# thethomasboyer/PhenDiff

Hardware: AMD Instinct MI355X
Metric: img2img images/sec (50-step DDIM invert+denoise, 256x256) (higher is better)
Workload: dtype bf16; 1 GPU; configs[2]: 256x256 pipeline_conditional_ddim invert->class-swap->denoise, 50+50 DDIM steps, super_small UNet (random init, seed 0), 3k_steps_clipping_rescaling, 32 images/GPU/step sharded over 1 GPU(s), no collectives; batch_per_gpu=32, global_batch=32, inference_steps=50, image_size=256, hipgraph=True, concurrent_trajectories=1

## Files before the change

### phendiff_amd/csrc/conv_igemm.hip

```cpp
#include <type_traits>
#include <utility>
#include <stdio.h>
#include <stdlib.h>
#include "pd_common.h"
#include "pd_stage.h"
#include "pd_conv.h"

namespace pd {

constexpr int CONV_AR8 = 6;
constexpr int CONV_PRO_DEFAULT = 1;
constexpr int CONV_PRO_WPS = 3;
constexpr int CONV_PRO_START = 8;
template <int... I, typename F> __device__ __forceinline__ void pd_static_for_impl(std::integer_sequence<int, I...>, F&& f) { (f(std::integral_constant<int, I>{}), ...); }
template <int N, typename F> __device__ __forceinline__ void pd_static_for(F&& f) { pd_static_for_impl(std::make_integer_sequence<int, N>{}, f); }
constexpr int PRO_OPS = 37;
constexpr int pro_op_cost(int k) {
  if (k >= 36) return 100;
  const int stg = (k % 18) >> 1;
  return (stg == 3 || stg == 4 || stg == 6 || stg == 7) ? 87 : (stg == 0 ? 60 : (stg == 8 ? 106 : 58));
}
constexpr int pro_ops_done(int S, int NS, int PS0, int NIT) {
  if (S < PS0) return 0;
  if (S >= NS - 1) return NIT * PRO_OPS;
  long long tot = 0;
  for (int k = 0; k < PRO_OPS; ++k) tot += pro_op_cost(k);
  tot *= NIT;
  const long long target = (long long)(S - PS0 + 1) * tot / (NS - PS0);
  int done = 0;
  long long dc = 0;
  while (done < NIT * PRO_OPS && dc + pro_op_cost(done % PRO_OPS) <= target) { dc += pro_op_cost(done % PRO_OPS); ++done; }
  return done;
}
__device__ __forceinline__ unsigned pd_lin_block() { return blockIdx.x + gridDim.x * (blockIdx.y + gridDim.y * blockIdx.z); }
template <typename T, int KS, int STRIDE, int TH, int TW, bool DB, bool TAIL, int NCO = 1, bool PLAIN = false, int PRO = 0, bool STACK = false>
__global__ __launch_bounds__(256, NCO == 2 ? 2 : (PRO ? CONV_PRO_WPS : (((KS == 1 || (KS == 3 && STRIDE == 1 && TH * TW == 256)) && sizeof(T) == 2) ? 3 : 2))) void conv_kernel(const ConvP p) {
  static_assert(PRO == 0 || (!PLAIN && DB && KS == 3 && STRIDE == 1 && sizeof(T) == 2), "compile-time prologue: 16-bit 3x3 stride-1 double-buffered launches");
  static_assert(!TAIL || (DB && KS == 3 && STRIDE == 1), "fused shortcut tail: 3x3 stride-1 double-buffered variant only");
  static_assert(NCO == 1 || (NCO == 2 && DB && KS == 3 && STRIDE == 1), "two output tiles per workgroup: 3x3 stride-1 double-buffered variant only");
  static_assert(!STACK || (KS == 3 && STRIDE == 1 && TW == 8 && TH == 16 && NCO == 1 && !PLAIN && PRO == 0), "stacked 8 x 8 images: the 16 x 8 tile");
  constexpr int SG = STACK ? TH / 8 : 1;
  using E = Elem<T>;
  using Frag = typename E::Frag;
  using SR = typename Stage<T>::R;
  constexpr int TP = TH * TW;
  constexpr int NF = TP / 64;
  constexpr int RPF = 32 / TW;
  constexpr int IN_TH = STACK ? SG * 10 : (TH - 1) * STRIDE + KS;
  constexpr int IN_TW = (TW - 1) * STRIDE + KS;
  constexpr int NPIX = IN_TH * IN_TW;
  constexpr bool M16 = PLAIN && sizeof(T) == 2 && (KS == 3 || KS == 2) && STRIDE == 1 && DB && TW >= 16;
  constexpr int CHB = 32 * E::BYTES;
  constexpr int PITCH = DB ? 2 * CHB + (M16 ? 32 : 16) : CHB + 16;
  constexpr int NIT = (NPIX * 4 + 255) / 256;
  constexpr int TAPS = KS * KS;
  constexpr int KSTEPS = TAPS * 2;
  constexpr int LDS_TILE = DB ? CHB : 0;
  static_assert(RPF >= 1 && TW * RPF == 32, "TW must divide 32");

  extern __shared__ __attribute__((aligned(16))) unsigned char lds[];

  int co_t = blockIdx.y, n = blockIdx.z * SG, bx = blockIdx.x;
  if (!STACK && p.co_major) {
    const int gx = gridDim.x, gxz = gridDim.x * gridDim.z;
    const int idx = xcd_chunk_index((int)pd_lin_block(), gxz * (int)gridDim.y);
    co_t = idx / gxz;
    const int rem = idx - co_t * gxz;
    n = rem / gx; bx = rem - n * gx;
  }
  int tx, ty;
  if (p.tiles_x_shift >= 0) { tx = bx & (p.tiles_x - 1); ty = bx >> p.tiles_x_shift; }
  else { ty = bx / p.tiles_x; tx = bx - ty * p.tiles_x; }
  const int y0 = ty * TH, x0 = tx * TW;

  const int tid = threadIdx.x;
  const int lane = tid & 63;
  const int wave = __builtin_amdgcn_readfirstlane(tid >> 6);
  const int wp = wave >> 1, wc = wave & 1;
  const int r = lane & 31, h = lane >> 5;
  const int ct32 = co_t * (2 * NCO) + wc;
  const bool wave_active = (ct32 * 32) < p.Cout_pad;

  const __amdgpu_buffer_rsrc_t rs0 = __builtin_amdgcn_make_buffer_rsrc((void*)p.x0, 0, p.bytes0, 0x00020000);
  const __amdgpu_buffer_rsrc_t rs1 = __builtin_amdgcn_make_buffer_rsrc((void*)(p.x1 ? p.x1 : p.x0), 0, p.bytes1, 0x00020000);

  const __amdgpu_buffer_rsrc_t rt0 = __builtin_amdgcn_make_buffer_rsrc((void*)(TAIL ? p.t0 : p.x0), 0, TAIL ? p.tbytes0 : p.bytes0, 0x00020000);
  const __amdgpu_buffer_rsrc_t rt1 = __builtin_amdgcn_make_buffer_rsrc((void*)((TAIL && p.t1) ? p.t1 : p.x0), 0, (TAIL && p.t1) ? p.tbytes1 : p.bytes0, 0x00020000);

  const int sub = tid & 3;
  auto stage_pix = [&](int i) { return (tid + 256 * i) >> 2; };
  const int Hc = p.upsample ? p.Hin * 2 : p.Hin;
  const int Wc = p.upsample ? p.Win * 2 : p.Win;
  int spix[NIT];
  constexpr int TAIL_CENTRE = 1 << 30;
  const int ups = p.upsample ? 1 : 0;
  const int ph_mask = p.upsample >= 2 ? 1 : 0, ph_want = p.upsample == 3 ? 1 : 0;
  const int istep = p.in_step, Ws = p.Win * istep;
  const int iy_base = y0 * STRIDE - p.pad, ix_base = x0 * STRIDE - p.pad_x, n_base = n * p.Hin * istep + p.in_oy;
#pragma unroll
  for (int i = 0; i < NIT; ++i) {
    const int pix = stage_pix(i);
    const int u = pix / IN_TW, vv = pix - u * IN_TW;
    const int sj = STACK ? u / 10 : 0, su = u - sj * 10;
    const int iy = STACK ? su - 1 : iy_base + u, ix = ix_base + vv;
    const bool ok = (pix < NPIX) & ((unsigned)iy < (unsigned)Hc) & ((unsigned)ix < (unsigned)Wc) & (!STACK || n + sj < p.B)
                    & (((iy & ph_mask) == (ph_want & ph_mask)) & ((ix & ph_mask) == (ph_want & ph_mask)));
    int v = STACK ? ((n + sj) * 8 + iy) * 8 + ix : (n_base + (iy >> ups) * istep) * Ws + (ix >> ups) * istep + p.in_ox;
    if (TAIL) v |= (((unsigned)((STACK ? su : u) - KS / 2) < (unsigned)(STACK ? 8 : TH)) & ((unsigned)(vv - KS / 2) < (unsigned)TW)) ? TAIL_CENTRE : 0;
    spix[i] = ok ? v : -1;
  }
  const bool affine = PRO || (!PLAIN && p.scale != nullptr);
  const bool do_silu = PRO || (!PLAIN && p.silu != 0);
  const int cin = p.C0 + p.C1;

  SR stage[NIT];
  float sc[8], sh[8];
  bool stage_plain = false;
  auto issue_loads = [&](int chunk) {
    int src, cch;
    if (!TAIL || chunk < p.n_main) { cch = chunk * 32; src = cch < p.C0 ? 0 : 1; if (src == 1) cch -= p.C0; }
    else { cch = (chunk - p.n_main) * 32; src = cch < p.Ct0 ? 2 : 3; if (src == 3) cch -= p.Ct0; }
    stage_plain = TAIL && src >= 2;
    const unsigned cs = src == 0 ? p.C0 : (src == 1 ? p.C1 : (src == 2 ? p.Ct0 : p.Ct1));
    const unsigned cbytes = (unsigned)(cch + sub * 8) * E::BYTES;
#pragma unroll
    for (int i = 0; i < NIT; ++i) {
      const bool want = TAIL ? (stage_plain ? spix[i] >= TAIL_CENTRE : spix[i] >= 0) : spix[i] >= 0;
      const unsigned off = want ? (unsigned)(TAIL ? spix[i] & (TAIL_CENTRE - 1) : spix[i]) * cs * E::BYTES + cbytes : OOB_OFF;
      stage[i] = src == 0 ? Stage<T>::load(rs0, off) : (src == 1 ? Stage<T>::load(rs1, off)
                 : (src == 2 ? Stage<T>::load(rt0, off) : Stage<T>::load(rt1, off)));
    }
    if ((PRO && !stage_plain) || (!PRO && affine && !stage_plain)) {
      const int cg = chunk * 32 + sub * 8;
      const float* ps = p.scale + (size_t)n * cin + cg;
      const float* pb = p.shift + (size_t)n * cin + cg;
      const f32x4 a0 = *(const f32x4*)ps, a1 = *((const f32x4*)ps + 1);
      const f32x4 b0 = *(const f32x4*)pb, b1 = *((const f32x4*)pb + 1);
#pragma unroll
      for (int j = 0; j < 4; ++j) { sc[j] = a0[j]; sc[4 + j] = a1[j]; sh[j] = b0[j]; sh[4 + j] = b1[j]; }
    }
  };
  auto write_piece = [&](int i, unsigned char* buf, bool tail_piece = false) {
    const int pix = stage_pix(i);
    if constexpr (PRO) {
      if (TAIL && tail_piece) {
        if (pix < NPIX && spix[i] >= 0) *(u32x4*)(buf + pix * PITCH + sub * 8 * E::BYTES) = Stage<T>::raw(stage[i]);
        return;
      }
      const u32x4 o = Stage<T>::xform_gs(stage[i], sc, sh);
      const bool ok = pix < NPIX && spix[i] >= 0;
      *(u32x4*)(ok ? buf + pix * PITCH + sub * 8 * E::BYTES : lds + NPIX * PITCH) = o;
    } else
    if (pix < NPIX && spix[i] >= 0)
      Stage<T>::template xform_store<false>(buf + pix * PITCH + sub * 8 * E::BYTES, stage[i], sc, sh, affine && !stage_plain,
                                            do_silu && !stage_plain, true);
  };
  auto zero_padding = [&]() {
#pragma unroll
    for (int i = 0; i < NIT; ++i) {
      const int pix = stage_pix(i);
      if (pix < NPIX && spix[i] < 0) {
        unsigned char* d = lds + pix * PITCH + sub * 8 * E::BYTES;
#pragma unroll
        for (int q = 0; q < (DB ? 2 : 1); ++q)
#pragma unroll
          for (int b16 = 0; b16 < 8 * E::BYTES; b16 += 16) *(u32x4*)(d + q * LDS_TILE + b16) = (u32x4)(0u);
      }
    }
  };

  auto stage_im2col = [&](unsigned char* buf) {
    if constexpr (KS == 1 && STRIDE == 1) {
      const int py = tid / TW, px = tid % TW;
      const int oy = y0 + py, ox = x0 + px;
// ... 17 lines not shown
      }
#pragma unroll
      for (int q = 0; q < 4; ++q) {
        float o[8];
#pragma unroll
        for (int j = 0; j < 8; ++j) o[j] = v[q * 8 + j];
        E::store(buf + tid * PITCH + q * 8 * E::BYTES, E::pack(o));
      }
    }
  };

  auto frag_row = [&](int fi, int q) { return fi * RPF + q; };
  const int li = lane & 15, lg = lane >> 4;
  constexpr int TJ_STEP = (TW >= 32 ? 16 : IN_TW) * PITCH;
  int rbase[NF];
#pragma unroll
  for (int f = 0; f < NF; ++f) {
    const int fi = wp * NF + f;
    if constexpr (M16) {
      rbase[f] = f == 0 ? ((wp * NF * RPF) * IN_TW + li) * PITCH + lg * 8 * E::BYTES : 0;
    } else {
      const int py = frag_row(fi, r / TW), px = r % TW;
      const int ly = STACK ? py + 2 * (py >> 3) : py * STRIDE;
      rbase[f] = (ly * IN_TW + px * STRIDE) * PITCH + h * 8 * E::BYTES;
    }
  }

  f32x16 acc[NCO][NF];
  f32x4 acq[NCO][NF][4];
  const int main_ksteps = (TAIL ? p.n_main : p.nchunks) * KSTEPS;
  const int all_ksteps = main_ksteps + (TAIL ? p.n_tail * 2 : 0);
  const unsigned wfrag = 512u * E::BYTES;
  const __amdgpu_buffer_rsrc_t rw = __builtin_amdgcn_make_buffer_rsrc((void*)p.w, 0, (unsigned)(p.Cout_pad / 32) * (unsigned)all_ksteps * wfrag, 0x00020000);
  const unsigned wlane = (unsigned)lane * 8u * E::BYTES;
  const unsigned wtile = (unsigned)ct32 * (unsigned)all_ksteps * wfrag;
  const unsigned wstep = 2u * (unsigned)all_ksteps * wfrag;
  auto load_w = [&](int c, int kstep) { return E::load_buf(rw, wlane, wtile + (unsigned)c * wstep + (unsigned)kstep * wfrag); };

  constexpr int AR = (KS == 3 && TW == 8 && STRIDE == 1 && sizeof(T) == 2 && TP <= 128) ? CONV_AR8 : ((KSTEPS % 3 == 0) ? 3 : 2);
  static_assert(KSTEPS % AR == 0, "the ring index is static");
  constexpr int AD = AR - 1;
  Frag aring[AR][NCO];
  static_assert(!M16 || NF % 2 == 0, "M16 walks a fragment pair per half-step");
  Frag aq[2][NCO][2];
  const unsigned wlane16 = (unsigned)(((lg >> 1) * 64 + (lg & 1) * 32 + li) * 16);
  auto load_w16 = [&](int c, int tap_index, int ti) {
    return E::load_buf(rw, wlane16 + (unsigned)ti * 256u, wtile + (unsigned)c * wstep + (unsigned)(2 * tap_index) * wfrag);
  };

  auto mma_chunk = [&](int chunk, const unsigned char* buf, unsigned char* nbuf, auto have_next_c, auto active_c) {
    constexpr int NEXT = (int)decltype(have_next_c)::value;
    constexpr bool HAVE_NEXT = NEXT != 0, NEXT_PLAIN = NEXT == 2;
    constexpr bool ACTIVE = decltype(active_c)::value;
    const int g0 = chunk * KSTEPS;
    Frag bc[NF];
    int piece = 0;
    if constexpr (!PRO) __builtin_amdgcn_iglp_opt(0);
    if constexpr (PRO && ACTIVE) {
      constexpr int NM = NCO * NF;
      constexpr int NS = KSTEPS * NM;
      constexpr int PS0 = CONV_PRO_START < NS - 8 ? CONV_PRO_START : 0;
      f32x2 py[4], pw[4];
      u32x4 po;
      auto piece_op = [&](auto ic, auto kc) __attribute__((always_inline)) {
        constexpr int i = decltype(ic)::value, k = decltype(kc)::value;
        if constexpr (k < 36) {
          constexpr int half = k / 18, kk = k % 18, stg = kk >> 1, j = half * 2 + (kk & 1);
          if constexpr (stg == 0) { const uint32_t wj = Stage<T>::word(stage[i], j); float lo, hi; Pack16<T>::unpack(wj, lo, hi); pw[j].x = lo; pw[j].y = hi; }
          else if constexpr (stg == 1) py[j] = pw[j] * (f32x2){sc[2 * j], sc[2 * j + 1]} + (f32x2){sh[2 * j], sh[2 * j + 1]};
          else if constexpr (stg == 2) pw[j] = py[j] * (f32x2)(-1.4426950408889634f);
          else if constexpr (stg == 3) pw[j].x = __builtin_amdgcn_exp2f(pw[j].x);
          else if constexpr (stg == 4) pw[j].y = __builtin_amdgcn_exp2f(pw[j].y);
          else if constexpr (stg == 5) pw[j] = pw[j] + (f32x2)(1.0f);
          else if constexpr (stg == 6) pw[j].x = __builtin_amdgcn_rcpf(pw[j].x);
          else if constexpr (stg == 7) pw[j].y = __builtin_amdgcn_rcpf(pw[j].y);
          else { const f32x2 o = py[j] * pw[j]; po[j] = Pack16<T>::pack(o.x, o.y); }
          if constexpr (stg == 1) asm volatile("" : "+v"(py[j]));
          else if constexpr (stg == 8) { uint32_t w = po[j]; asm volatile("" : "+v"(w)); po[j] = w; }
          else asm volatile("" : "+v"(pw[j]));
        } else {
// ... 145 lines not shown
  };
  using std::true_type; using std::false_type;

  f32x4 bt[NCO][4];
  u32x4 tv[NCO][4];
  if constexpr (M16) {
    if (wave_active) {
      const __amdgpu_buffer_rsrc_t rtemb = __builtin_amdgcn_make_buffer_rsrc((void*)(p.temb ? p.temb : p.bias), 0,
          p.temb ? ((unsigned)n * (unsigned)p.temb_stride + (unsigned)p.Cout) * 4u : 0u, 0x00020000);
#pragma unroll
      for (int c = 0; c < NCO; ++c)
#pragma unroll
        for (int ti = 0; ti < 2; ++ti) {
          const int co = (ct32 + 2 * c) * 32 + 16 * ti + 4 * lg;
          bt[c][ti] = *(const f32x4*)(p.bias + co);
          tv[c][ti] = __builtin_amdgcn_raw_buffer_load_b128(rtemb, (unsigned)(n * p.temb_stride + co) * 4u, 0, 0);
        }
    }
  } else
  if (wave_active) {
    const int nt = STACK ? min(n + wp, p.B - 1) : n;
    const __amdgpu_buffer_rsrc_t rtemb = __builtin_amdgcn_make_buffer_rsrc((void*)(p.temb ? p.temb : p.bias), 0,
        p.temb ? ((unsigned)nt * (unsigned)p.temb_stride + (unsigned)p.Cout) * 4u : 0u, 0x00020000);
#pragma unroll
    for (int c = 0; c < NCO; ++c)
#pragma unroll
      for (int g = 0; g < 4; ++g) {
        const int co = (ct32 + 2 * c) * 32 + 8 * g + 4 * h;
        bt[c][g] = *(const f32x4*)(p.bias + co);
        tv[c][g] = __builtin_amdgcn_raw_buffer_load_b128(rtemb, (unsigned)(nt * p.temb_stride + co) * 4u, 0, 0);
      }
  }
  if (!p.im2col3) issue_loads(0);
  if (wave_active) {
#pragma unroll
    for (int c = 0; c < NCO; ++c)
#pragma unroll
      for (int g = 0; g < (M16 ? 2 : 4); ++g)
#pragma unroll
        for (int i = 0; i < 4; ++i) bt[c][g][i] += __uint_as_float(tv[c][g][i]);
  }
  if constexpr (M16) {
#pragma unroll
    for (int c = 0; c < NCO; ++c)
#pragma unroll
      for (int f = 0; f < NF; ++f)
#pragma unroll
        for (int q = 0; q < 4; ++q) acq[c][f][q] = wave_active ? bt[c][q >> 1] : (f32x4)(0.f);
    if (wave_active) {
#pragma unroll
      for (int c = 0; c < NCO; ++c) { aq[0][c][0] = load_w16(c, 0, 0); aq[0][c][1] = load_w16(c, 0, 1); }
    }
  } else {
#pragma unroll
  for (int c = 0; c < NCO; ++c) {
    f32x16 init = (f32x16)(0.f);
    if (wave_active) {
#pragma unroll
      for (int g = 0; g < 4; ++g)
#pragma unroll
        for (int i = 0; i < 4; ++i) init[4 * g + i] = bt[c][g][i];
    }
#pragma unroll
    for (int f = 0; f < NF; ++f) acc[c][f] = init;
  }
  if (wave_active) {
#pragma unroll
    for (int i = 0; i < AD; ++i)
#pragma unroll
      for (int c = 0; c < NCO; ++c) aring[i][c] = load_w(c, i);
  }
  }
  if (!p.im2col3) zero_padding();
  if (DB) {
    if (p.im2col3) {
      stage_im2col(lds);
    } else {
      write_piece(0, lds);
#pragma unroll
      for (int i = 1; i < NIT; ++i) write_piece(i, lds);
    }
    if (p.nchunks > 1) issue_loads(1);
    __syncthreads();
    int chunk = 0;
    const int main_loop_end = TAIL ? (PRO ? p.n_main - 1 : p.n_main) : p.nchunks - 1;
    for (; chunk < main_loop_end; ++chunk) {
      unsigned char* buf = lds + (chunk & 1) * LDS_TILE;
      unsigned char* nbuf = lds + ((chunk + 1) & 1) * LDS_TILE;
      if constexpr (PRO) mma_chunk(chunk, buf, nbuf, true_type{}, true_type{});
      else if (wave_active) mma_chunk(chunk, buf, nbuf, true_type{}, true_type{});
      else mma_chunk(chunk, buf, nbuf, true_type{}, false_type{});
      if (chunk + 2 < p.nchunks) issue_loads(chunk + 2);
      __syncthreads();
    }
    if constexpr (TAIL && PRO) {
      mma_chunk(chunk, lds + (chunk & 1) * LDS_TILE, lds + ((chunk + 1) & 1) * LDS_TILE, std::integral_constant<int, 2>{}, true_type{});
      if (chunk + 2 < p.nchunks) issue_loads(chunk + 2);
      __syncthreads();
      ++chunk;
    }
    if constexpr (TAIL) {
      for (; chunk + 1 < p.nchunks; ++chunk) {
        unsigned char* buf = lds + (chunk & 1) * LDS_TILE;
        unsigned char* nbuf = lds + ((chunk + 1) & 1) * LDS_TILE;
        if (wave_active) mma_tail(chunk, buf, nbuf, true_type{}, true_type{});
        else mma_tail(chunk, buf, nbuf, true_type{}, false_type{});
// ... 161 lines not shown
      *(u32x4*)((T*)p.y + ((((size_t)which * p.B + n) * p.heads + (cc >> 3)) * N + tok) * 8 + (cc & 7)) = v;
    }
  }
  if (p.stats) {
    float* red = (float*)(lds + TP * EP_PITCH);
#pragma unroll
    for (int sg = 0; sg < SG; ++sg) {
      if (sg > 0) __syncthreads();
#pragma unroll
      for (int q = 0; q < 2 * EPC / 4; ++q) {
        f32x4 v4;
#pragma unroll
        for (int j = 0; j < 4; ++j) { const int e = q * 4 + j; v4[j] = e < EPC ? ssum[sg][e] : ssq[sg][e - EPC]; }
        *(f32x4*)(red + tid * (2 * EPC) + q * 4) = v4;
      }
      __syncthreads();
      if (tid < 128) {
        const int c = tid >> 1, which = tid & 1;
        const int pc = c / EPC, j = c % EPC;
        const int cog = co_tile * 64 + c;
        float tot = 0.f;
#pragma unroll 8
        for (int pr = 0; pr < PXI; ++pr) tot += red[(pr * PPP + pc) * (2 * EPC) + which * EPC + j];
        if (cog < p.Cout && n + sg < p.B) {
          const int tile = p.stat_tile_base + ty * p.tiles_x + tx;
          p.stats[(((size_t)(n + sg) * p.stat_tiles + tile) * p.Cout + cog) * 2 + which] = tot;
        }
      }
    }
  }
  }
}

template <typename T, int KS, int STRIDE, int TH, int TW, bool TAIL = false, int NCO = 1, bool PLAIN = false, int PRO = 0, bool STACK = false>
static int launch_conv(const ConvP& p, hipStream_t st) {
  constexpr int IN_TH = STACK ? (TH / 8) * 10 : (TH - 1) * STRIDE + KS, IN_TW = (TW - 1) * STRIDE + KS;
  constexpr int PITCH = 32 * Elem<T>::BYTES + 16;
  constexpr int LDS_TILE = ((IN_TH * IN_TW * PITCH + 15) / 16) * 16;
  constexpr bool DB = 2 * LDS_TILE <= 100 * 1024 && STRIDE != 2;
  constexpr bool M16 = PLAIN && sizeof(T) == 2 && (KS == 3 || KS == 2) && STRIDE == 1 && TW >= 16;
  constexpr int LDS_DB = ((IN_TH * IN_TW * (2 * 32 * Elem<T>::BYTES + (M16 ? 32 : 16)) + 15) / 16) * 16;
  constexpr int EPI_BYTES = TH * TW * (64 * Elem<T>::BYTES + 16) + 256 * 64;
  constexpr int LDS_MAIN = (DB ? LDS_DB : LDS_TILE) + (PRO ? 16 : 0);
  constexpr int LDS_BYTES = LDS_MAIN > EPI_BYTES ? LDS_MAIN : EPI_BYTES;
  static_assert(LDS_BYTES <= 160 * 1024, "tile too large");
  static_assert(NCO == 1 || DB, "NCO = 2 is a double-buffered variant");
  auto kern = conv_kernel<T, KS, STRIDE, TH, TW, DB, TAIL, NCO, PLAIN, PRO, STACK>;
  if (LDS_BYTES > 64 * 1024) {
    static LdsAttr attr;
    if (!ensure_lds(attr, kern, LDS_BYTES)) { set_error("pd_conv: cannot reserve %d bytes of LDS", LDS_BYTES); return PD_ERR_LAUNCH; }
  }
  ConvP q = p;
  q.tiles_x = (p.Wout + TW - 1) / TW;
  q.tiles_y = STACK ? 1 : (p.Hout + TH - 1) / TH;
  q.tiles_x_shift = -1;
  for (int sft = 0; sft < 16; ++sft) if ((1 << sft) == q.tiles_x) q.tiles_x_shift = sft;
  q.n_co_tiles = (p.Cout_pad + 63) / 64;
  if (q.stat_tiles == 0) q.stat_tiles = q.tiles_x * q.tiles_y;
  else { q.stat_tiles *= q.tiles_x * q.tiles_y; q.stat_tile_base *= q.tiles_x * q.tiles_y; }
  {
    const long long es = (long long)sizeof(T), cin = (long long)p.C0 + p.C1;
    const long long wbytes = (long long)p.Cout_pad * cin * KS * KS * es, abytes = (long long)p.B * p.Hin * p.Win * cin * es;
    const long long blocks = (long long)q.tiles_x * q.tiles_y * (q.n_co_tiles / NCO) * p.B;
    const int env = diag_env("PD_CONV_XCD", 0);
    q.co_major = !STACK && blocks >= 64 && blocks < (1ll << 30) && !p.im2col3 && (env == 1 || (env == 2 && wbytes > abytes));
  }
  hipLaunchKernelGGL(kern, dim3(q.tiles_x * q.tiles_y, q.n_co_tiles / NCO, STACK ? (p.B + TH / 8 - 1) / (TH / 8) : p.B), dim3(256), LDS_BYTES, st, q);
  PD_LAUNCH_CHECK();
  return PD_OK;
}

static void tile_shape(int ksize, int stride, int hout, int wout, int* th, int* tw) {
  const int tp = (ksize == 3 && stride == 1 && wout <= 8 && hout <= 8) ? 64
                 : ((ksize == 3 && stride == 2) || (ksize == 3 && stride == 1 && wout < 16 && hout <= 16)) ? 128 : 256;
  *tw = wout >= 32 ? 32 : (wout >= 16 ? 16 : 8);
  *th = tp / *tw;
}

template <typename T>
static int dispatch_conv(const ConvP& p, int ksize, int stride, hipStream_t st) {
  const int w = p.Wout;
  if (ksize == 3 && stride == 1) {
    const bool tiny = p.Hout <= 16;
    if constexpr (sizeof(T) == 2) {
      const int nco_env = diag_env("PD_CONV_NCO", 0);
      static int cus_of[16] = {0};
      int dev = 0;
      if (hipGetDevice(&dev) != hipSuccess || dev < 0 || dev >= 16) dev = 0;
      if (cus_of[dev] == 0) {
        int c = 0;
        if (hipDeviceGetAttribute(&c, hipDeviceAttributeMultiprocessorCount, dev) != hipSuccess || c <= 0) c = 256;
        cus_of[dev] = c;
      }
      const int cus = cus_of[dev];
      bool nco2 = false;
      if (w >= 32 && p.Cout_pad % 128 == 0 && p.Cout == p.Cout_pad && p.out_mode != PD_OUT_NCHW_F32) {
        const long long wgs1 = (long long)((p.Wout + 31) / 32) * ((p.Hout + 7) / 8) * (p.Cout_pad / 64) * p.B, wgs2 = wgs1 / 2;
        auto eff = [](long long wgs, long long slots) { return (double)wgs / (double)(((wgs + slots - 1) / slots) * slots); };
        const double speed2 = (p.scale != nullptr && p.C0 + p.C1 >= 128) ? 1.05 : 0.84;
        nco2 = nco_env ? nco_env == 2 : eff(wgs2, 2ll * cus) * speed2 > eff(wgs1, 3ll * cus);
      }
      const bool plain_off = diag_env("PD_CONV_PLAIN", 1) == 0;
      const bool plain = !plain_off && p.scale == nullptr && !p.silu && !p.im2col3 && w >= 16;
      const int pro_lvl = diag_env("PD_CONV_PRO", CONV_PRO_DEFAULT);
      const bool gs = p.scale != nullptr && p.silu != 0 && !p.im2col3 && w >= 32 && p.Cout_pad % 64 == 0 && p.out_mode != PD_OUT_NCHW_F32;
      if (nco2 && gs && pro_lvl >= 1)
        return p.n_tail > 0 ? launch_conv<T, 3, 1, 8, 32, true, 2, false, 1>(p, st) : launch_conv<T, 3, 1, 8, 32, false, 2, false, 1>(p, st);
      if (nco2) return p.n_tail > 0 ? launch_conv<T, 3, 1, 8, 32, true, 2>(p, st) : launch_conv<T, 3, 1, 8, 32, false, 2>(p, st);
      if (plain) {
        if (p.n_tail > 0) return w >= 32 ? launch_conv<T, 3, 1, 8, 32, true, 1, true>(p, st) : launch_conv<T, 3, 1, 16, 16, true, 1, true>(p, st);
        return w >= 32 ? launch_conv<T, 3, 1, 8, 32, false, 1, true>(p, st) : launch_conv<T, 3, 1, 16, 16, false, 1, true>(p, st);
      }
    }
    const bool one8 = p.Hout <= 8 && w <= 8;
    const bool stack = p.Hout == 8 && w == 8 && p.Hin == 8 && p.Win == 8 && !p.upsample && p.in_step == 1 && p.out_step == 1 && p.pad == 1 && p.pad_x == 1 &&
                       p.scale == nullptr && !p.silu && !p.im2col3 && p.out_mode == PD_OUT_NHWC && p.B >= 2 && diag_env("PD_CONV_STACK", 0) != 0;
    if (stack) return p.n_tail > 0 ? launch_conv<T, 3, 1, 16, 8, true, 1, false, 0, true>(p, st) : launch_conv<T, 3, 1, 16, 8, false, 1, false, 0, true>(p, st);
    if (p.n_tail > 0) {
      if (w >= 32) return launch_conv<T, 3, 1, 8, 32, true>(p, st);
      if (w >= 16) return launch_conv<T, 3, 1, 16, 16, true>(p, st);
      if (one8) return launch_conv<T, 3, 1, 8, 8, true>(p, st);
      if (tiny) return launch_conv<T, 3, 1, 16, 8, true>(p, st);
      return launch_conv<T, 3, 1, 32, 8, true>(p, st);
    }
    if (w >= 32) return launch_conv<T, 3, 1, 8, 32>(p, st);
    if (w >= 16) return launch_conv<T, 3, 1, 16, 16>(p, st);
    if (one8) return launch_conv<T, 3, 1, 8, 8>(p, st);
    if (tiny) return launch_conv<T, 3, 1, 16, 8>(p, st);
    return launch_conv<T, 3, 1, 32, 8>(p, st);
  }
  if (ksize == 3 && stride == 2) {
    if (w >= 32) return launch_conv<T, 3, 2, 4, 32>(p, st);
    if (w >= 16) return launch_conv<T, 3, 2, 8, 16>(p, st);
    return launch_conv<T, 3, 2, 16, 8>(p, st);
  }
  if (ksize == 2 && stride == 1) {
    if (w >= 32) return launch_conv<T, 2, 1, 8, 32, false, 1, true>(p, st);
    if (w >= 16) return launch_conv<T, 2, 1, 16, 16, false, 1, true>(p, st);
    set_error("pd_conv: the 2x2 phase form needs Wout >= 16");
    return PD_ERR_UNSUPPORTED;
  }
  if (ksize == 1 && stride == 1) {
    if (w >= 32) return launch_conv<T, 1, 1, 8, 32>(p, st);
    if (w >= 16) return launch_conv<T, 1, 1, 16, 16>(p, st);
    return launch_conv<T, 1, 1, 32, 8>(p, st);
  }
  set_error("pd_conv: unsupported ksize=%d stride=%d", ksize, stride);
  return PD_ERR_UNSUPPORTED;
}

}

extern "C" int pd_conv(const pd_conv_args* a, void* stream) {
  using namespace pd;
  PD_CHECK(a != nullptr, PD_ERR_ARG, "pd_conv: null args");
  PD_CHECK(a->dtype == PD_F32 || a->dtype == PD_BF16 || a->dtype == PD_F16, PD_ERR_ARG, "pd_conv: bad dtype %d", a->dtype);
  PD_CHECK(a->B > 0 && a->Hin > 0 && a->Win > 0 && a->Hout > 0 && a->Wout > 0, PD_ERR_SHAPE, "pd_conv: bad spatial shape");
  PD_CHECK(a->C0 > 0 && a->C0 % 32 == 0 && a->C1 >= 0 && a->C1 % 32 == 0, PD_ERR_SHAPE,
           "pd_conv: C0=%d C1=%d must be multiples of 32", a->C0, a->C1);
  PD_CHECK(a->Cout > 0 && a->Cout_pad >= a->Cout && a->Cout_pad % 32 == 0, PD_ERR_SHAPE, "pd_conv: bad Cout/Cout_pad");
  PD_CHECK(a->Cout % 8 == 0 || a->out_mode == PD_OUT_NCHW_F32, PD_ERR_SHAPE, "pd_conv: NHWC / head-major output needs Cout %% 8 == 0");
  PD_CHECK(a->x0 && a->w_packed && a->bias && a->y, PD_ERR_ARG, "pd_conv: null pointer");
  PD_CHECK((a->C1 == 0) == (a->x1 == nullptr), PD_ERR_ARG, "pd_conv: x1/C1 mismatch");
  PD_CHECK((a->scale == nullptr) == (a->shift == nullptr), PD_ERR_ARG, "pd_conv: scale/shift mismatch");
// ... 79 lines not shown
```

### phendiff_amd/csrc/pd_conv.h

```cpp
#pragma once
#include "pd_common.h"

namespace pd {

struct ConvP {
  int B, Hin, Win, Hout, Wout;
  int C0, C1, Cout, Cout_pad;
  int pad, upsample, silu, out_mode, heads;
  int tiles_x, tiles_y, tiles_x_shift, n_co_tiles, nchunks;
  unsigned bytes0, bytes1;
  const void* x0; const void* x1;
  const float* scale; const float* shift;
  const void* w;
  const float* bias;
  const float* temb; int temb_stride;
  const void* residual;
  void* y;
  float* stats;
  int n_main, n_tail, Ct0, Ct1;
  unsigned tbytes0, tbytes1;
  const void* t0; const void* t1;
  int im2col3;
  int C0r;
  int pad_x, out_step, out_oy, out_ox, stat_tile_base, stat_tiles;
  int in_step, in_oy, in_ox;
  int co_major;
};

}
```

### phendiff_amd/csrc/small_kernels.hip

```cpp
#include <stdarg.h>
#include <stdio.h>
#include "pd_common.h"
#include "pd_guided.h"

namespace pd {

static thread_local char g_err[512] = "";
void set_error(const char* fmt, ...) {
  va_list ap;
  va_start(ap, fmt);
  vsnprintf(g_err, sizeof(g_err), fmt, ap);
  va_end(ap);
}

__global__ __launch_bounds__(256) void temb_kernel(const pd_temb_args a, int skip_proj) {
  extern __shared__ float sm[];
  float* se = sm;
  float* h1 = sm + a.c0;
  float* act = h1 + a.tdim;
  const int row = blockIdx.x, tid = threadIdx.x;
  const float t = a.timesteps[row];
  const int half = a.c0 / 2;
  const bool first = blockIdx.y == 0;
  for (int i = tid; i < a.c0; i += 256) {
// ... 207 lines not shown
    part[sl][cl][0] = s; part[sl][cl][1] = q;
    __syncthreads();
    if (sl == 0 && c < c_hi) {
      double ts = 0.0, tq = 0.0;
#pragma unroll
      for (int k = 0; k < 16; ++k) { ts += part[k][cl][0]; tq += part[k][cl][1]; }
      chs[c - c_lo] = ts; chq[c - c_lo] = tq;
    }
    __syncthreads();
  }
  const int gs = C / a.groups;
  const int g_lo = c_lo / gs, ng = (c_hi - c_lo) / gs;
  if (tid < ng) {
    double ds = 0.0, dq = 0.0;
    for (int c = tid * gs; c < (tid + 1) * gs; ++c) { ds += chs[c]; dq += chq[c]; }
    const double cnt = (double)gs * (double)a.HW;
    const double mean = ds / cnt;
    double var = dq / cnt - mean * mean;
    if (var < 0.0) var = 0.0;
    mean_s[tid] = (float)mean;
    rstd_s[tid] = (float)(1.0 / sqrt(var + (double)a.eps));
    if (a.mean) { a.mean[n * a.groups + g_lo + tid] = mean_s[tid]; a.rstd[n * a.groups + g_lo + tid] = rstd_s[tid]; }
  }
  __syncthreads();
  for (int c = c_lo + tid; c < c_hi; c += 1024) {
    const int g = c / gs - g_lo;
    const float sc = rstd_s[g] * a.gamma[c];
    gn_write_affine(a, n, C, c, sc, a.beta[c] - mean_s[g] * sc);
  }
}

__global__ __launch_bounds__(1024) void gn_finalize3_kernel(const pd_gn_finalize_args a, int CB, int CBp) {
  __shared__ double ps[1024], pq[1024];
  __shared__ float mean_s[16], rstd_s[16];
  const int C = a.C0 + a.C1;
  const int n = blockIdx.x, tid = threadIdx.x;
  const int c_lo = blockIdx.y * CB, c_hi = min(C, c_lo + CB);
  const int cl = tid & (CBp - 1), sl = tid / CBp, S = 1024 / CBp;
  const int c = c_lo + cl;
  double s = 0.0, q = 0.0;
  if (cl < CB && c < c_hi) {
    const bool first = c < a.C0;
    const float* st = first ? a.stats0 : a.stats1;
    const int Cs = first ? a.C0 : a.C1, T = first ? a.T0 : a.T1, cc = first ? c : c - a.C0;
    const float* base = st + ((size_t)n * T * Cs + cc) * 2;
#pragma unroll 4
    for (int t = sl; t < T; t += S) {
      const float2 v = *(const float2*)(base + (size_t)t * Cs * 2);
      s += (double)v.x; q += (double)v.y;
    }
  }
  ps[tid] = s; pq[tid] = q;
  __syncthreads();
  for (int off = S >> 1; off > 0; off >>= 1) {
    if (sl < off) { ps[tid] += ps[tid + off * CBp]; pq[tid] += pq[tid + off * CBp]; }
    __syncthreads();
  }
  const int gs = C / a.groups;
  const int g_lo = c_lo / gs, ng = (c_hi - c_lo) / gs;
  if (tid < ng) {
    double ds = 0.0, dq = 0.0;
    for (int k = tid * gs; k < (tid + 1) * gs; ++k) { ds += ps[k]; dq += pq[k]; }
    const double cnt = (double)gs * (double)a.HW;
    const double mean = ds / cnt;
    double var = dq / cnt - mean * mean;
    if (var < 0.0) var = 0.0;
    mean_s[tid] = (float)mean;
    rstd_s[tid] = (float)(1.0 / sqrt(var + (double)a.eps));
    if (a.mean) { a.mean[n * a.groups + g_lo + tid] = mean_s[tid]; a.rstd[n * a.groups + g_lo + tid] = rstd_s[tid]; }
  }
  __syncthreads();
  if (tid < c_hi - c_lo) {
    const int cc = c_lo + tid;
    const int g = tid / gs;
    const float sc = rstd_s[g] * a.gamma[cc];
    gn_write_affine(a, n, C, cc, sc, a.beta[cc] - mean_s[g] * sc);
  }
}

__global__ __launch_bounds__(256) void ddim_step_kernel(const pd_ddim_step_args a) {
#pragma clang fp contract(off)
  const int64_t i0 = ((int64_t)blockIdx.x * 256 + threadIdx.x) * 4;
  if (i0 >= a.numel) return;
  const int cnt = (int)min((int64_t)4, a.numel - i0);
  float x[4], o[4], u[4], xp[4], x0v[4];
  if (cnt == 4) {
    f32x4 vx = *(const f32x4*)(a.sample + i0), vo = *(const f32x4*)(a.model_out + i0);
#pragma unroll
    for (int j = 0; j < 4; ++j) { x[j] = vx[j]; o[j] = vo[j]; }
    if (a.uncond_out) { f32x4 vu = *(const f32x4*)(a.uncond_out + i0);
#pragma unroll
      for (int j = 0; j < 4; ++j) u[j] = vu[j]; }
  } else {
    for (int j = 0; j < 4; ++j) { x[j] = j < cnt ? a.sample[i0 + j] : 0.f; o[j] = j < cnt ? a.model_out[i0 + j] : 0.f;
      u[j] = (a.uncond_out && j < cnt) ? a.uncond_out[i0 + j] : 0.f; }
  }
#pragma unroll
  for (int j = 0; j < 4; ++j) {
    float out = o[j];
    if (a.uncond_out) {
      const float w = a.w_per_sample ? a.w[(i0 + (j < cnt ? j : 0)) / a.per_sample] : a.w[0];
      out = a.guidance_cfg ? (o[j] + w * (o[j] - u[j])) : (u[j] + w * (o[j] - u[j]));
    }
    xp[j] = ddim_step_elem(a, x[j], out, x0v[j]);
  }
  if (cnt == 4) {
    *(f32x4*)(a.prev_sample + i0) = (f32x4){xp[0], xp[1], xp[2], xp[3]};
    if (a.pred_x0) *(f32x4*)(a.pred_x0 + i0) = (f32x4){x0v[0], x0v[1], x0v[2], x0v[3]};
  } else {
// ... 200 lines not shown
```

Baseline: 17.00 images/s.

## Add streaming conv variants for 32-channel 3x3 and stride-2 downsample layers

Adds a STREAM template form of the implicit-GEMM conv. The stride-1 8x32 form targets layers with 64 input channels and 32 output channels. It gives each of the four waves one pixel band over the single 32-wide output tile, loads both input chunks up front, stages them to LDS together, and runs the two MMA chunks without double-buffer handoffs. Weight loads are masked for rows past Cout. The stride-2 4x32 form uses a deeper weight ring (AR=9) and 3 waves-per-SIMD launch bounds for 64/128-channel downsamples. The aim is to cut serialization and idle waves on small-channel layers, at the cost of higher register pressure and added dispatch complexity.

```diff
diff --git a/phendiff_amd/csrc/conv_igemm.hip b/phendiff_amd/csrc/conv_igemm.hip
--- a/phendiff_amd/csrc/conv_igemm.hip
+++ b/phendiff_amd/csrc/conv_igemm.hip
@@ -12,6 +12,8 @@
 constexpr int CONV_PRO_DEFAULT = 1;
 constexpr int CONV_PRO_WPS = 3;
 constexpr int CONV_PRO_START = 8;
+constexpr int CONV_STREAM_DEFAULT = 1;
+constexpr int CONV_STREAM_AR = 9;
 template <int... I, typename F> __device__ __forceinline__ void pd_static_for_impl(std::integer_sequence<int, I...>, F&& f) { (f(std::integral_constant<int, I>{}), ...); }
 template <int N, typename F> __device__ __forceinline__ void pd_static_for(F&& f) { pd_static_for_impl(std::make_integer_sequence<int, N>{}, f); }
 constexpr int PRO_OPS = 37;
@@ -33,8 +35,11 @@
   return done;
 }
 __device__ __forceinline__ unsigned pd_lin_block() { return blockIdx.x + gridDim.x * (blockIdx.y + gridDim.y * blockIdx.z); }
-template <typename T, int KS, int STRIDE, int TH, int TW, bool DB, bool TAIL, int NCO = 1, bool PLAIN = false, int PRO = 0, bool STACK = false>
-__global__ __launch_bounds__(256, NCO == 2 ? 2 : (PRO ? CONV_PRO_WPS : (((KS == 1 || (KS == 3 && STRIDE == 1 && TH * TW == 256)) && sizeof(T) == 2) ? 3 : 2))) void conv_kernel(const ConvP p) {
+template <typename T, int KS, int STRIDE, int TH, int TW, bool DB, bool TAIL, int NCO = 1, bool PLAIN = false, int PRO = 0, bool STACK = false, bool STREAM = false>
+__global__ __launch_bounds__(256, STREAM ? 3 : (NCO == 2 ? 2 : (PRO ? CONV_PRO_WPS : (((KS == 1 || (KS == 3 && STRIDE == 1 && TH * TW == 256)) && sizeof(T) == 2) ? 3 : 2)))) void conv_kernel(const ConvP p) {
+  static_assert(!STREAM || (sizeof(T) == 2 && KS == 3 && !TAIL && NCO == 1 && PRO == 0 && !STACK && TW == 32 && ((STRIDE == 1 && DB && TH == 8) || (STRIDE == 2 && !DB && !PLAIN && TH == 4))),
+                "streaming forms: 16-bit 3x3 launches, the 8 x 32 stride-1 tile or the 4 x 32 stride-2 tile");
+  constexpr bool STREAM1 = STREAM && STRIDE == 1;
   static_assert(PRO == 0 || (!PLAIN && DB && KS == 3 && STRIDE == 1 && sizeof(T) == 2), "compile-time prologue: 16-bit 3x3 stride-1 double-buffered launches");
   static_assert(!TAIL || (DB && KS == 3 && STRIDE == 1), "fused shortcut tail: 3x3 stride-1 double-buffered variant only");
   static_assert(NCO == 1 || (NCO == 2 && DB && KS == 3 && STRIDE == 1), "two output tiles per workgroup: 3x3 stride-1 double-buffered variant only");
@@ -44,7 +49,7 @@
   using Frag = typename E::Frag;
   using SR = typename Stage<T>::R;
   constexpr int TP = TH * TW;
-  constexpr int NF = TP / 64;
+  constexpr int NF = STREAM1 ? TP / 128 : TP / 64;
   constexpr int RPF = 32 / TW;
   constexpr int IN_TH = STACK ? SG * 10 : (TH - 1) * STRIDE + KS;
   constexpr int IN_TW = (TW - 1) * STRIDE + KS;
@@ -76,7 +81,7 @@
   const int tid = threadIdx.x;
   const int lane = tid & 63;
   const int wave = __builtin_amdgcn_readfirstlane(tid >> 6);
-  const int wp = wave >> 1, wc = wave & 1;
+  const int wp = STREAM1 ? wave : wave >> 1, wc = STREAM1 ? 0 : wave & 1;
   const int r = lane & 31, h = lane >> 5;
   const int ct32 = co_t * (2 * NCO) + wc;
   const bool wave_active = (ct32 * 32) < p.Cout_pad;
@@ -115,8 +120,11 @@
 
   SR stage[NIT];
   float sc[8], sh[8];
+  SR stage1[STREAM1 ? NIT : 1];
+  float sc1[8], sh1[8];
   bool stage_plain = false;
-  auto issue_loads = [&](int chunk) {
+  auto issue_loads_to = [&](int chunk, auto second_c) {
+    constexpr bool SECOND = decltype(second_c)::value;
     int src, cch;
     if (!TAIL || chunk < p.n_main) { cch = chunk * 32; src = cch < p.C0 ? 0 : 1; if (src == 1) cch -= p.C0; }
     else { cch = (chunk - p.n_main) * 32; src = cch < p.Ct0 ? 2 : 3; if (src == 3) cch -= p.Ct0; }
@@ -127,8 +135,9 @@
     for (int i = 0; i < NIT; ++i) {
       const bool want = TAIL ? (stage_plain ? spix[i] >= TAIL_CENTRE : spix[i] >= 0) : spix[i] >= 0;
       const unsigned off = want ? (unsigned)(TAIL ? spix[i] & (TAIL_CENTRE - 1) : spix[i]) * cs * E::BYTES + cbytes : OOB_OFF;
-      stage[i] = src == 0 ? Stage<T>::load(rs0, off) : (src == 1 ? Stage<T>::load(rs1, off)
-                 : (src == 2 ? Stage<T>::load(rt0, off) : Stage<T>::load(rt1, off)));
+      const SR v = src == 0 ? Stage<T>::load(rs0, off) : (src == 1 ? Stage<T>::load(rs1, off)
+                   : (src == 2 ? Stage<T>::load(rt0, off) : Stage<T>::load(rt1, off)));
+      if constexpr (SECOND) stage1[i] = v; else stage[i] = v;
     }
     if ((PRO && !stage_plain) || (!PRO && affine && !stage_plain)) {
       const int cg = chunk * 32 + sub * 8;
@@ -137,9 +146,13 @@
       const f32x4 a0 = *(const f32x4*)ps, a1 = *((const f32x4*)ps + 1);
       const f32x4 b0 = *(const f32x4*)pb, b1 = *((const f32x4*)pb + 1);
 #pragma unroll
-      for (int j = 0; j < 4; ++j) { sc[j] = a0[j]; sc[4 + j] = a1[j]; sh[j] = b0[j]; sh[4 + j] = b1[j]; }
+      for (int j = 0; j < 4; ++j) {
+        if constexpr (SECOND) { sc1[j] = a0[j]; sc1[4 + j] = a1[j]; sh1[j] = b0[j]; sh1[4 + j] = b1[j]; }
+        else { sc[j] = a0[j]; sc[4 + j] = a1[j]; sh[j] = b0[j]; sh[4 + j] = b1[j]; }
+      }
     }
   };
+  auto issue_loads = [&](int chunk) { issue_loads_to(chunk, std::false_type{}); };
   auto write_piece = [&](int i, unsigned char* buf, bool tail_piece = false) {
     const int pix = stage_pix(i);
     if constexpr (PRO) {
@@ -223,12 +236,13 @@
   const int all_ksteps = main_ksteps + (TAIL ? p.n_tail * 2 : 0);
   const unsigned wfrag = 512u * E::BYTES;
   const __amdgpu_buffer_rsrc_t rw = __builtin_amdgcn_make_buffer_rsrc((void*)p.w, 0, (unsigned)(p.Cout_pad / 32) * (unsigned)all_ksteps * wfrag, 0x00020000);
-  const unsigned wlane = (unsigned)lane * 8u * E::BYTES;
+  const int wrows = STREAM1 ? p.Cout - ct32 * 32 : 32;
+  const unsigned wlane = r < wrows ? (unsigned)lane * 8u * E::BYTES : OOB_OFF;
   const unsigned wtile = (unsigned)ct32 * (unsigned)all_ksteps * wfrag;
   const unsigned wstep = 2u * (unsigned)all_ksteps * wfrag;
   auto load_w = [&](int c, int kstep) { return E::load_buf(rw, wlane, wtile + (unsigned)c * wstep + (unsigned)kstep * wfrag); };
 
-  constexpr int AR = (KS == 3 && TW == 8 && STRIDE == 1 && sizeof(T) == 2 && TP <= 128) ? CONV_AR8 : ((KSTEPS % 3 == 0) ? 3 : 2);
+  constexpr int AR = STREAM ? CONV_STREAM_AR : (KS == 3 && TW == 8 && STRIDE == 1 && sizeof(T) == 2 && TP <= 128) ? CONV_AR8 : ((KSTEPS % 3 == 0) ? 3 : 2);
   static_assert(KSTEPS % AR == 0, "the ring index is static");
   constexpr int AD = AR - 1;
   Frag aring[AR][NCO];
@@ -236,7 +250,7 @@
   Frag aq[2][NCO][2];
   const unsigned wlane16 = (unsigned)(((lg >> 1) * 64 + (lg & 1) * 32 + li) * 16);
   auto load_w16 = [&](int c, int tap_index, int ti) {
-    return E::load_buf(rw, wlane16 + (unsigned)ti * 256u, wtile + (unsigned)c * wstep + (unsigned)(2 * tap_index) * wfrag);
+    return E::load_buf(rw, 16 * ti + li < wrows ? wlane16 + (unsigned)ti * 256u : OOB_OFF, wtile + (unsigned)c * wstep + (unsigned)(2 * tap_index) * wfrag);
   };
 
   auto mma_chunk = [&](int chunk, const unsigned char* buf, unsigned char* nbuf, auto have_next_c, auto active_c) {
@@ -448,6 +462,7 @@
       }
   }
   if (!p.im2col3) issue_loads(0);
+  if constexpr (STREAM1) issue_loads_to(1, true_type{});
   if (wave_active) {
 #pragma unroll
     for (int c = 0; c < NCO; ++c)
@@ -488,6 +503,20 @@
   }
   }
   if (!p.im2col3) zero_padding();
+  if constexpr (STREAM1) {
+#pragma unroll
+    for (int i = 0; i < NIT; ++i) write_piece(i, lds);
+#pragma unroll
+    for (int i = 0; i < NIT; ++i) {
+      const int pix = stage_pix(i);
+      if (pix < NPIX && spix[i] >= 0)
+        Stage<T>::template xform_store<false>(lds + LDS_TILE + pix * PITCH + sub * 8 * E::BYTES, stage1[i], sc1, sh1, affine, do_silu, true);
+    }
+    __syncthreads();
+    mma_chunk(0, lds, lds, false_type{}, true_type{});
+    mma_chunk(1, lds + LDS_TILE, lds, false_type{}, true_type{});
+    __syncthreads();
+  } else
   if (DB) {
     if (p.im2col3) {
       stage_im2col(lds);
@@ -715,7 +744,7 @@
   }
 }
 
-template <typename T, int KS, int STRIDE, int TH, int TW, bool TAIL = false, int NCO = 1, bool PLAIN = false, int PRO = 0, bool STACK = false>
+template <typename T, int KS, int STRIDE, int TH, int TW, bool TAIL = false, int NCO = 1, bool PLAIN = false, int PRO = 0, bool STACK = false, bool STREAM = false>
 static int launch_conv(const ConvP& p, hipStream_t st) {
   constexpr int IN_TH = STACK ? (TH / 8) * 10 : (TH - 1) * STRIDE + KS, IN_TW = (TW - 1) * STRIDE + KS;
   constexpr int PITCH = 32 * Elem<T>::BYTES + 16;
@@ -728,7 +757,7 @@
   constexpr int LDS_BYTES = LDS_MAIN > EPI_BYTES ? LDS_MAIN : EPI_BYTES;
   static_assert(LDS_BYTES <= 160 * 1024, "tile too large");
   static_assert(NCO == 1 || DB, "NCO = 2 is a double-buffered variant");
-  auto kern = conv_kernel<T, KS, STRIDE, TH, TW, DB, TAIL, NCO, PLAIN, PRO, STACK>;
+  auto kern = conv_kernel<T, KS, STRIDE, TH, TW, DB, TAIL, NCO, PLAIN, PRO, STACK, STREAM>;
   if (LDS_BYTES > 64 * 1024) {
     static LdsAttr attr;
     if (!ensure_lds(attr, kern, LDS_BYTES)) { set_error("pd_conv: cannot reserve %d bytes of LDS", LDS_BYTES); return PD_ERR_LAUNCH; }
@@ -787,6 +816,9 @@
       const bool plain = !plain_off && p.scale == nullptr && !p.silu && !p.im2col3 && w >= 16;
       const int pro_lvl = diag_env("PD_CONV_PRO", CONV_PRO_DEFAULT);
       const bool gs = p.scale != nullptr && p.silu != 0 && !p.im2col3 && w >= 32 && p.Cout_pad % 64 == 0 && p.out_mode != PD_OUT_NCHW_F32;
+      if (diag_env("PD_CONV_STREAM", CONV_STREAM_DEFAULT) != 0 && p.nchunks == 2 && p.n_tail == 0 && p.Cout_pad == 32 && w >= 32 && !p.im2col3 &&
+          !p.upsample && p.in_step == 1 && p.out_step == 1 && p.out_mode != PD_OUT_QKV_HEADS)
+        return plain ? launch_conv<T, 3, 1, 8, 32, false, 1, true, 0, false, true>(p, st) : launch_conv<T, 3, 1, 8, 32, false, 1, false, 0, false, true>(p, st);
       if (nco2 && gs && pro_lvl >= 1)
         return p.n_tail > 0 ? launch_conv<T, 3, 1, 8, 32, true, 2, false, 1>(p, st) : launch_conv<T, 3, 1, 8, 32, false, 2, false, 1>(p, st);
       if (nco2) return p.n_tail > 0 ? launch_conv<T, 3, 1, 8, 32, true, 2>(p, st) : launch_conv<T, 3, 1, 8, 32, false, 2>(p, st);
@@ -813,6 +845,10 @@
     return launch_conv<T, 3, 1, 32, 8>(p, st);
   }
   if (ksize == 3 && stride == 2) {
+    if constexpr (sizeof(T) == 2) {
+      if (w >= 32 && diag_env("PD_CONV_STREAM", CONV_STREAM_DEFAULT) != 0 && p.C0 + p.C1 == p.Cout && p.Cout == p.Cout_pad && (p.Cout == 64 || p.Cout == 128))
+        return launch_conv<T, 3, 2, 4, 32, false, 1, false, 0, false, true>(p, st);
+    }
     if (w >= 32) return launch_conv<T, 3, 2, 4, 32>(p, st);
     if (w >= 16) return launch_conv<T, 3, 2, 8, 16>(p, st);
     return launch_conv<T, 3, 2, 16, 8>(p, st);
```

New measurement: 11.58 images/s. 31.9% lower.

## Add specialized output conv kernel and wave-shuffle GroupNorm finalize reduction

Applied to the files above, without the earlier changes.

Adds a dedicated 3x3 conv kernel for the final output layer (64 input channels, 32 padded outputs, GroupNorm+SiLU prologue, fp32 NCHW output). It uses a 9-deep weight ring, a fixed 8x32 tile and bias+temb folded into the accumulator init, and the dispatcher routes matching convs to it by default. Separately, gn_finalize3 now finishes its reduction with wave shuffles instead of LDS loops and barriers. It also prefetches gamma/beta/temb and writes scale/shift inline, folding in the temb scale-shift. The changes aim to cut launch-bound latency in the last conv and in GN finalize, at the risk of replacing the gn_write_affine path with inline logic.

```diff
diff --git a/phendiff_amd/csrc/conv_edge.hip b/phendiff_amd/csrc/conv_edge.hip
--- /dev/null
+++ b/phendiff_amd/csrc/conv_edge.hip
@@ -0,0 +1,144 @@
+#include "pd_common.h"
+#include "pd_stage.h"
+#include "pd_conv.h"
+
+namespace pd {
+
+constexpr int EDGE_AR = 9;
+
+template <typename T>
+__global__ __launch_bounds__(256, 3) void conv_out_kernel(const ConvP p) {
+  using E = Elem<T>;
+  using Frag = typename E::Frag;
+  using SR = typename Stage<T>::R;
+  static_assert(E::BYTES == 2, "16-bit engines");
+  constexpr int TH = 8, TW = 32, IN_TW = TW + 2, NPIX = (TH + 2) * IN_TW;
+  constexpr int PITCH = 2 * 32 * E::BYTES + 16;
+  constexpr int NIT = (NPIX * 8 + 255) / 256;
+  constexpr int KSTEPS = 36, AR = EDGE_AR, AD = AR - 1;
+  static_assert(KSTEPS % AR == 0, "the ring index is static");
+
+  extern __shared__ __attribute__((aligned(16))) unsigned char lds[];
+
+  const int n = blockIdx.z, bx = blockIdx.x;
+  int tx, ty;
+  if (p.tiles_x_shift >= 0) { tx = bx & (p.tiles_x - 1); ty = bx >> p.tiles_x_shift; }
+  else { ty = bx / p.tiles_x; tx = bx - ty * p.tiles_x; }
+  const int y0 = ty * TH, x0 = tx * TW;
+  const int tid = threadIdx.x;
+  const int lane = tid & 63;
+  const int wave = __builtin_amdgcn_readfirstlane(tid >> 6);
+  const int r = lane & 31, h = lane >> 5;
+
+  const __amdgpu_buffer_rsrc_t rtemb = __builtin_amdgcn_make_buffer_rsrc((void*)(p.temb ? p.temb : p.bias), 0,
+      p.temb ? ((unsigned)n * (unsigned)p.temb_stride + (unsigned)p.Cout) * 4u : 0u, 0x00020000);
+  f32x4 bt[4];
+  u32x4 tv[4];
+#pragma unroll
+  for (int g = 0; g < 4; ++g) {
+    const int co = 8 * g + 4 * h;
+    bt[g] = *(const f32x4*)(p.bias + co);
+    tv[g] = __builtin_amdgcn_raw_buffer_load_b128(rtemb, (unsigned)(n * p.temb_stride + co) * 4u, 0, 0);
+  }
+  const int sub = tid & 7;
+  float sc[8], sh[8];
+  {
+    const float* ps = p.scale + (size_t)n * 64 + sub * 8;
+    const float* pb = p.shift + (size_t)n * 64 + sub * 8;
+    const f32x4 a0 = *(const f32x4*)ps, a1 = *((const f32x4*)ps + 1);
+    const f32x4 b0 = *(const f32x4*)pb, b1 = *((const f32x4*)pb + 1);
+#pragma unroll
+    for (int j = 0; j < 4; ++j) { sc[j] = a0[j]; sc[4 + j] = a1[j]; sh[j] = b0[j]; sh[4 + j] = b1[j]; }
+  }
+  const __amdgpu_buffer_rsrc_t rs0 = __builtin_amdgcn_make_buffer_rsrc((void*)p.x0, 0, p.bytes0, 0x00020000);
+  const int pix0 = tid >> 3;
+  SR stage[NIT];
+  unsigned okm = 0;
+  {
+    int u = 0, v = pix0;
+    const int iy_base = y0 - p.pad, ix_base = x0 - p.pad_x;
+#pragma unroll
+    for (int i = 0; i < NIT; ++i) {
+      const int iy = iy_base + u, ix = ix_base + v;
+      const bool ok = (pix0 + 32 * i < NPIX) & ((unsigned)iy < (unsigned)p.Hin) & ((unsigned)ix < (unsigned)p.Win);
+      const unsigned off = ok ? (unsigned)((n * p.Hin + iy) * p.Win + ix) * (64u * E::BYTES) + (unsigned)sub * 16u : OOB_OFF;
+      stage[i] = Stage<T>::load(rs0, off);
+      okm |= ok ? (1u << i) : 0u;
+      v += 32;
+      if (v >= IN_TW) { v -= IN_TW; ++u; }
+    }
+  }
+  const unsigned wfrag = 512u * E::BYTES;
+  const __amdgpu_buffer_rsrc_t rw = __builtin_amdgcn_make_buffer_rsrc((void*)p.w, 0, (unsigned)KSTEPS * wfrag, 0x00020000);
+  const unsigned wlane = (unsigned)lane * 8u * E::BYTES;
+  auto load_w = [&](int kstep) { return E::load_buf(rw, wlane, (unsigned)kstep * wfrag); };
+  Frag aring[AR];
+#pragma unroll
+  for (int i = 0; i < AD; ++i) aring[i] = load_w(i);
+
+  f32x16 acc[2];
+  {
+    f32x16 init;
+#pragma unroll
+    for (int g = 0; g < 4; ++g)
+#pragma unroll
+      for (int i = 0; i < 4; ++i) init[4 * g + i] = bt[g][i] + __uint_as_float(tv[g][i]);
+    acc[0] = init; acc[1] = init;
+  }
+#pragma unroll
+  for (int i = 0; i < NIT; ++i) {
+    if (pix0 + 32 * i < NPIX) {
+      u32x4 o = Stage<T>::xform_gs(stage[i], sc, sh);
+      if (!((okm >> i) & 1u)) o = (u32x4)(0u);
+      *(u32x4*)(lds + (pix0 + 32 * i) * PITCH + sub * 16) = o;
+    }
+  }
+  __syncthreads();
+
+  int rbase[2];
+#pragma unroll
+  for (int f = 0; f < 2; ++f) rbase[f] = ((2 * wave + f) * IN_TW + r) * PITCH + h * 8 * E::BYTES;
+#pragma unroll
+  for (int g = 0; g < KSTEPS; ++g) {
+    const int chunk = g / 18, ks = g % 18, tap = ks >> 1, s = ks & 1;
+    const int toff = ((tap / 3) * IN_TW + (tap % 3)) * PITCH + chunk * 32 * E::BYTES + s * 16 * E::BYTES;
+    aring[(g + AD) % AR] = load_w(g + AD);
+    Frag b[2];
+#pragma unroll
+    for (int f = 0; f < 2; ++f) b[f] = E::load(lds + rbase[f] + toff);
+    __builtin_amdgcn_s_setprio(1);
+#pragma unroll
+    for (int f = 0; f < 2; ++f) acc[f] = E::mma(aring[g % AR], b[f], acc[f]);
+    __builtin_amdgcn_s_setprio(0);
+  }
+
+#pragma unroll
+  for (int f = 0; f < 2; ++f) {
+    const int oy = y0 + 2 * wave + f, ox = x0 + r;
+    if (oy >= p.Hout || ox >= p.Wout) continue;
+#pragma unroll
+    for (int g = 0; g < 4; ++g) {
+      const int co = 8 * g + 4 * h;
+#pragma unroll
+      for (int i = 0; i < 4; ++i)
+        if (co + i < p.Cout) ((float*)p.y)[(((size_t)n * p.Cout + co + i) * p.Hout + oy) * p.Wout + ox] = acc[f][4 * g + i];
+    }
+  }
+}
+
+template <typename T>
+int launch_conv_out(const ConvP& p, hipStream_t st) {
+  constexpr int LDS_BYTES = 10 * 34 * 144;
+  ConvP q = p;
+  q.tiles_x = (p.Wout + 31) / 32;
+  q.tiles_y = (p.Hout + 7) / 8;
+  q.tiles_x_shift = -1;
+  for (int sft = 0; sft < 16; ++sft) if ((1 << sft) == q.tiles_x) q.tiles_x_shift = sft;
+  hipLaunchKernelGGL(conv_out_kernel<T>, dim3(q.tiles_x * q.tiles_y, 1, p.B), dim3(256), LDS_BYTES, st, q);
+  PD_LAUNCH_CHECK();
+  return PD_OK;
+}
+template int launch_conv_out<bf16_t>(const ConvP&, hipStream_t);
+template int launch_conv_out<half_t>(const ConvP&, hipStream_t);
+
+}
diff --git a/phendiff_amd/csrc/conv_igemm.hip b/phendiff_amd/csrc/conv_igemm.hip
--- a/phendiff_amd/csrc/conv_igemm.hip
+++ b/phendiff_amd/csrc/conv_igemm.hip
@@ -766,6 +766,9 @@
   if (ksize == 3 && stride == 1) {
     const bool tiny = p.Hout <= 16;
     if constexpr (sizeof(T) == 2) {
+      if (p.C0 == 64 && p.C1 == 0 && p.n_tail == 0 && !p.upsample && !p.im2col3 && p.in_step == 1 && p.out_step == 1 && p.scale != nullptr && p.silu != 0 &&
+          p.out_mode == PD_OUT_NCHW_F32 && p.Cout_pad == 32 && w >= 32 && diag_env("PD_CONV_EDGE", 1) != 0)
+        return launch_conv_out<T>(p, st);
       const int nco_env = diag_env("PD_CONV_NCO", 0);
       static int cus_of[16] = {0};
       int dev = 0;
diff --git a/phendiff_amd/csrc/pd_conv.h b/phendiff_amd/csrc/pd_conv.h
--- a/phendiff_amd/csrc/pd_conv.h
+++ b/phendiff_amd/csrc/pd_conv.h
@@ -27,4 +27,6 @@
   int co_major;
 };
 
+template <typename T> int launch_conv_out(const ConvP& p, hipStream_t st);
+
 }
diff --git a/phendiff_amd/csrc/small_kernels.hip b/phendiff_amd/csrc/small_kernels.hip
--- a/phendiff_amd/csrc/small_kernels.hip
+++ b/phendiff_amd/csrc/small_kernels.hip
@@ -263,12 +263,17 @@
 
 __global__ __launch_bounds__(1024) void gn_finalize3_kernel(const pd_gn_finalize_args a, int CB, int CBp) {
   __shared__ double ps[1024], pq[1024];
-  __shared__ float mean_s[16], rstd_s[16];
   const int C = a.C0 + a.C1;
   const int n = blockIdx.x, tid = threadIdx.x;
   const int c_lo = blockIdx.y * CB, c_hi = min(C, c_lo + CB);
   const int cl = tid & (CBp - 1), sl = tid / CBp, S = 1024 / CBp;
   const int c = c_lo + cl;
+  const bool row = tid < c_hi - c_lo;
+  float gam = 0.f, bet = 0.f, t_sc = 0.f, t_sh = 0.f;
+  if (row) {
+    gam = a.gamma[c_lo + tid]; bet = a.beta[c_lo + tid];
+    if (a.temb) { const float* tr = a.temb + (size_t)n * a.temb_stride; t_sc = tr[c_lo + tid]; t_sh = tr[C + c_lo + tid]; }
+  }
   double s = 0.0, q = 0.0;
   if (cl < CB && c < c_hi) {
     const bool first = c < a.C0;
@@ -283,29 +288,37 @@
   }
   ps[tid] = s; pq[tid] = q;
   __syncthreads();
-  for (int off = S >> 1; off > 0; off >>= 1) {
+  int off = S >> 1;
+  for (; off * CBp > 64; off >>= 1) {
     if (sl < off) { ps[tid] += ps[tid + off * CBp]; pq[tid] += pq[tid + off * CBp]; }
     __syncthreads();
   }
+  if (tid >= 64) return;
+  s = ps[tid] + ps[tid + 64]; q = pq[tid] + pq[tid + 64];
+  for (int d = 32; d >= CBp; d >>= 1) { s += __shfl_down(s, d); q += __shfl_down(q, d); }
   const int gs = C / a.groups;
   const int g_lo = c_lo / gs, ng = (c_hi - c_lo) / gs;
-  if (tid < ng) {
-    double ds = 0.0, dq = 0.0;
-    for (int k = tid * gs; k < (tid + 1) * gs; ++k) { ds += ps[k]; dq += pq[k]; }
-    const double cnt = (double)gs * (double)a.HW;
-    const double mean = ds / cnt;
-    double var = dq / cnt - mean * mean;
-    if (var < 0.0) var = 0.0;
-    mean_s[tid] = (float)mean;
-    rstd_s[tid] = (float)(1.0 / sqrt(var + (double)a.eps));
-    if (a.mean) { a.mean[n * a.groups + g_lo + tid] = mean_s[tid]; a.rstd[n * a.groups + g_lo + tid] = rstd_s[tid]; }
-  }
-  __syncthreads();
-  if (tid < c_hi - c_lo) {
+  double ds = 0.0, dq = 0.0;
+  for (int j = 0; j < gs; ++j) { const int k = (tid * gs + j) & 63; ds += __shfl(s, k); dq += __shfl(q, k); }
+  const double cnt = (double)gs * (double)a.HW;
+  const double mean = ds / cnt;
+  double var = dq / cnt - mean * mean;
+  if (var < 0.0) var = 0.0;
+  const float mean_f = (float)mean, rstd_f = (float)(1.0 / sqrt(var + (double)a.eps));
+  if (tid < ng && a.mean) { a.mean[n * a.groups + g_lo + tid] = mean_f; a.rstd[n * a.groups + g_lo + tid] = rstd_f; }
+  const int g = (tid / gs) & 63;
+  const float mean_g = __shfl(mean_f, g), rstd_g = __shfl(rstd_f, g);
+  if (row) {
     const int cc = c_lo + tid;
-    const int g = tid / gs;
-    const float sc = rstd_s[g] * a.gamma[cc];
-    gn_write_affine(a, n, C, cc, sc, a.beta[cc] - mean_s[g] * sc);
+    float sc = rstd_g * gam;
+    float sh = bet - mean_g * sc;
+    if (a.temb) {
+      const float ts = 1.0f + t_sc;
+      sc *= ts;
+      sh = sh * ts + t_sh;
+    }
+    a.scale[(size_t)n * C + cc] = sc;
+    a.shift[(size_t)n * C + cc] = sh;
   }
 }
 
```

New measurement: 15.91 images/s before, 15.93 images/s after, median of 4. About the same (+0.1%).
